# USTC3DV/D3Human-code

Measured on AMD Instinct MI355X. Metric: train iters/sec @ tet-res 128, 1024^2 render; 1/2/4/8 MI355X, higher is better.
Workload: dtype f32; 1 GPU; config3: 4-frame batch, tet-res 128 (Kuhn n=63: 262144 verts / 1500282 tets), 1024x1024, mask+normal+SSIM+sdf_reg+eikonal; frames_per_gpu=4, mesh_faces=8626, parallelism=frame-parallel dp1

## Files before the change

d3human-code_amd/csrc/raster.hip:

```cpp
#include "d3h_common.h"
#include "composite.h"

namespace {

struct TriSetup {
    float X[3], Y[3], q[3], zw[3];
    bool ok;
    bool cross;
};

__device__ __forceinline__ TriSetup load_tri(const float* __restrict__ pos, const int* __restrict__ tri, int f) {
    TriSetup t;
    int nfront = 0;
#pragma unroll
    for (int k = 0; k < 3; ++k) {
        int vi = tri[3 * (size_t)f + k];
        float4 p = *(const float4*)(pos + 4 * (size_t)vi);
        if (p.w > 1e-8f) ++nfront;
        float w = (fabsf(p.w) < 1e-8f) ? ((p.w < 0.f) ? -1e-8f : 1e-8f) : p.w;
        float q = 1.0f / w;
        t.q[k] = q;
        t.X[k] = p.x * q;
        t.Y[k] = p.y * q;
        t.zw[k] = p.z * q;
    }
    t.ok = nfront == 3;
    t.cross = nfront == 1 || nfront == 2;
    return t;
}

__device__ __forceinline__ void edge_fn(const TriSetup& t, float fx, float fy, float (&a)[3]) {
    float x0 = t.X[0] - fx, y0 = t.Y[0] - fy, x1 = t.X[1] - fx, y1 = t.Y[1] - fy, x2 = t.X[2] - fx, y2 = t.Y[2] - fy;
// ... 767 lines not shown
    if (gg.g_face && d_face) {
        float* df = d_face + (size_t)b * face_bstride + (size_t)f * fw;
        for (int c = 0; c < fw; ++c) {
            float gc = hit ? gg.g_face[i * fw + c] : 0.f;
            float s = d3h_seg_sum(gc * u, lane, sg.start) + d3h_seg_sum(gc * v, lane, sg.start) + d3h_seg_sum(gc * (1.0f - u - v), lane, sg.start);
            if (sg.tail && hit && s != 0.f) atomicAdd(df + c, s);
        }
    }
    if (d_rast && inb) *(float4*)(d_rast + 4 * i) = make_float4(gu, gv, 0.f, 0.f);
    if (RAST) {
        const bool live = hit && !(gu == 0.f && gv == 0.f);
        if (__ballot(live) == 0ull) return;
        float out[9] = {0.f, 0.f, 0.f, 0.f, 0.f, 0.f, 0.f, 0.f, 0.f};
        int vi[3];
        if (live) {
            const int rem = (int)(i % npix_per_b);
            raster_bwd_pixel(pos + (size_t)b * pos_bstride, tri, f, rem % W, rem / W, H, W, gu, gv, out, vi);
        }
#pragma unroll
        for (int k = 0; k < 3; ++k) {
            const float sx = d3h_seg_sum(out[3 * k + 0], lane, sg.start);
            const float sy = d3h_seg_sum(out[3 * k + 1], lane, sg.start);
            const float sw = d3h_seg_sum(out[3 * k + 2], lane, sg.start);
            if (sg.tail && hit && (sx != 0.f || sy != 0.f || sw != 0.f)) {
                float* dp = d_pos + (size_t)b * pos_bstride + 4 * (size_t)tri[3 * (size_t)f + k];
                atomicAdd(dp + 0, sx);
                atomicAdd(dp + 1, sy);
                atomicAdd(dp + 3, sw);
            }
        }
    }
}

__device__ __forceinline__ unsigned hash64(unsigned long long k) {
    k ^= k >> 33; k *= 0xff51afd7ed558ccdull; k ^= k >> 33; k *= 0xc4ceb9fe1a85ec53ull; k ^= k >> 33;
    return (unsigned)k;
}

__global__ void aa_hash_build_kernel(const int* __restrict__ tri, int nf, unsigned long long* __restrict__ keys, int* __restrict__ vals, unsigned mask) {
    int i = blockIdx.x * blockDim.x + threadIdx.x;
    if (i >= 3 * nf) return;
    int f = i / 3, e = i % 3;
    int va = tri[3 * (size_t)f + e], vb = tri[3 * (size_t)f + (e + 1) % 3], vo = tri[3 * (size_t)f + (e + 2) % 3];
    if (va == vb) return;
    unsigned long long key = ((unsigned long long)(unsigned)min(va, vb) << 32) | (unsigned)max(va, vb);
    unsigned slot = hash64(key) & mask;
    for (unsigned probe = 0; probe <= mask; ++probe) {
        unsigned long long prev = atomicCAS(&keys[slot], ~0ull, key);
        if (prev == ~0ull || prev == key) {
            if (atomicCAS(&vals[2 * slot], -1, vo) != -1) atomicCAS(&vals[2 * slot + 1], -1, vo);
            return;
        }
        slot = (slot + 1) & mask;
    }
}

__device__ __forceinline__ int hash_other(const unsigned long long* __restrict__ keys, const int* __restrict__ vals, unsigned mask, int va, int vb,
                                          int vo) {
    unsigned long long key = ((unsigned long long)(unsigned)min(va, vb) << 32) | (unsigned)max(va, vb);
    unsigned slot = hash64(key) & mask;
    for (unsigned probe = 0; probe <= mask; ++probe) {
        unsigned long long k = keys[slot];
        if (k == key) {
            int o0 = vals[2 * slot], o1 = vals[2 * slot + 1];
            if (o1 == -1) return -1;
            return (o0 == vo) ? o1 : o0;
// ... 700 lines not shown
                       idx, nidx, n, npb, out, out_da);
    D3H_LAUNCH_CHECK();
    return D3H_OK;
}

extern "C" int d3h_interpolate_bwd_da(const float* attr, int attr_bstride, int na, const float* rast, const int* tri, const float* db,
                                      const int* idx, int nidx, const float* g_out, const float* g_da, int nb, int H, int W, float* d_attr,
                                      float* d_rast, float* d_db, void* stream) {
    if (nb < 0 || H < 0 || W < 0 || na < 0 || nidx < 0 || (!idx && nidx != na) || (g_da && !db)) return D3H_ERR_ARG;
    size_t npb = (size_t)H * W, n = npb * nb;
    if (n == 0) return D3H_OK;
    if (!rast) return D3H_ERR_ARG;
    hipLaunchKernelGGL(interp_bwd_da_kernel, dim3(d3h_cdiv(n, 256)), dim3(256), 0, (hipStream_t)stream, attr, attr_bstride, na, rast, tri, db,
                       idx, nidx, g_out, g_da, n, npb, d_attr, d_rast, d_db);
    D3H_LAUNCH_CHECK();
    return D3H_OK;
}

extern "C" int d3h_gbuffer_fwd(const float* attr, int attr_bstride, int na, const float* face_attr, int face_bstride, int fw, const float* rast,
                               const int* tri, int nb, int H, int W, float* out0, int w0, float* out1, int w1, float* out2, int w2, float* out3,
                               int w3, float* face_out, float* mask_out, void* stream) {
    if (w0 < 0 || w1 < 0 || w2 < 0 || w3 < 0 || w0 + w1 + w2 + w3 != na || (face_out && (!face_attr || fw <= 0))) return D3H_ERR_ARG;
    size_t npb = (size_t)H * W, n = npb * nb;
    if (n == 0) return D3H_OK;
    GbufOut o{{out0, out1, out2, out3}, {w0, w1, w2, w3}, face_out, mask_out};
    const int kt_ = d3h_ktime_begin(D3H_KT_GBUFFER_FWD, (long long)n, (hipStream_t)stream);
    hipLaunchKernelGGL(gbuffer_fwd_kernel, dim3(d3h_cdiv(n, 256)), dim3(256), 0, (hipStream_t)stream, attr, attr_bstride, na, face_attr,
                       face_bstride, fw, rast, tri, n, npb, o);
    d3h_ktime_end(kt_, (hipStream_t)stream);
    D3H_LAUNCH_CHECK();
    return D3H_OK;
}

extern "C" int d3h_gbuffer_bwd(const float* attr, int attr_bstride, int na, int face_bstride, int fw, const float* rast, const int* tri, int nb,
                               int H, int W, const float* g0, int w0, const float* g1, int w1, const float* g2, int w2, const float* g3, int w3,
                               const float* g_face, float* d_attr, float* d_face, float* d_rast, void* stream) {
    if (w0 < 0 || w1 < 0 || w2 < 0 || w3 < 0 || w0 + w1 + w2 + w3 != na) return D3H_ERR_ARG;
    size_t npb = (size_t)H * W, n = npb * nb;
    if (n == 0) return D3H_OK;
    GbufGrad gg{{g0, g1, g2, g3}, {w0, w1, w2, w3}, g_face};
    const int kt = d3h_ktime_begin(D3H_KT_GBUFFER_BWD, (long long)n, (hipStream_t)stream);
    hipLaunchKernelGGL((gbuffer_bwd_kernel<false>), dim3(d3h_cdiv(n, 256)), dim3(256), 0, (hipStream_t)stream, attr, attr_bstride, na, face_bstride, fw,
                       rast, tri, n, npb, gg, d_attr, d_face, d_rast, (const float*)nullptr, 0, H, W, (float*)nullptr);
    d3h_ktime_end(kt, (hipStream_t)stream);
    D3H_LAUNCH_CHECK();
    return D3H_OK;
}

extern "C" int d3h_gbuffer_raster_bwd(const float* attr, int attr_bstride, int na, int face_bstride, int fw, const float* rast, const int* tri, int nb,
                                      int H, int W, const float* g0, int w0, const float* g1, int w1, const float* g2, int w2, const float* g3, int w3,
                                      const float* g_face, float* d_attr, float* d_face, const float* pos, int pos_bstride, float* d_pos,
                                      void* stream) {
    if (w0 < 0 || w1 < 0 || w2 < 0 || w3 < 0 || w0 + w1 + w2 + w3 != na || !pos || !d_pos) return D3H_ERR_ARG;
    size_t npb = (size_t)H * W, n = npb * nb;
    if (n == 0) return D3H_OK;
    GbufGrad gg{{g0, g1, g2, g3}, {w0, w1, w2, w3}, g_face};
    const int kt = d3h_ktime_begin(D3H_KT_GBUFFER_BWD, (long long)n, (hipStream_t)stream);
    hipLaunchKernelGGL((gbuffer_bwd_kernel<true>), dim3(d3h_cdiv(n, 256)), dim3(256), 0, (hipStream_t)stream, attr, attr_bstride, na, face_bstride, fw,
                       rast, tri, n, npb, gg, d_attr, d_face, (float*)nullptr, pos, pos_bstride, H, W, d_pos);
    d3h_ktime_end(kt, (hipStream_t)stream);
    D3H_LAUNCH_CHECK();
    return D3H_OK;
}

extern "C" int d3h_antialias_hash(const int* tri, int nf, unsigned long long* keys, int* vals, int cap, void* stream) {
    if (cap <= 0 || (cap & (cap - 1))) return D3H_ERR_ARG;
    hipStream_t s = (hipStream_t)stream;
    const int kt_ = d3h_ktime_begin(D3H_KT_AA_PREP, (long long)(nf), (hipStream_t)(stream));
    if ((const char*)vals == (const char*)keys + (size_t)cap * 8) {
        (void)hipMemsetAsync(keys, 0xFF, (size_t)cap * 16, s);
    } else {
        (void)hipMemsetAsync(keys, 0xFF, (size_t)cap * 8, s);
        (void)hipMemsetAsync(vals, 0xFF, (size_t)cap * 8, s);
    }
    if (nf > 0) hipLaunchKernelGGL(aa_hash_build_kernel, dim3(d3h_cdiv(3 * (int64_t)nf, 256)), dim3(256), 0, s, tri, nf, keys, vals, (unsigned)(cap - 1));
    d3h_ktime_end(kt_, (hipStream_t)(stream));
    D3H_LAUNCH_CHECK();
    return D3H_OK;
}

extern "C" int d3h_antialias_flags(const float* pos, int pos_bstride, const int* tri, int nf, int nb, const unsigned long long* keys,
                                   const int* vals, int cap, int H, int W, unsigned char* flags, void* stream) {
    if (cap <= 0 || (cap & (cap - 1))) return D3H_ERR_ARG;
    if (nf <= 0 || nb <= 0) return D3H_OK;
    hipLaunchKernelGGL(aa_edge_flags_kernel, dim3(d3h_cdiv((int64_t)nf * nb, 256)), dim3(256), 0, (hipStream_t)stream, pos, pos_bstride, tri, nf, nb,
                       keys, vals, (unsigned)(cap - 1), H, W, flags);
    D3H_LAUNCH_CHECK();
    return D3H_OK;
}

extern "C" int d3h_antialias_fwd(const float* color, const float* rast, const float* pos, int pos_bstride, const int* tri, int nf,
                                 const unsigned char* flags, int nb, int H, int W, int C, float* out, void* stream) {
// ... 83 lines not shown
```

d3human-code_amd/csrc/texmlp.hip:

```cpp
#include <cstdlib>
#include "d3h_common.h"
#include "d3h_h2.h"

namespace {

constexpr int NL = 5, NF = 2, ENC = NL * NF;
constexpr int HID = 32, OUTC = 6;
constexpr int W1N = HID * ENC, W2N = HID * HID, W3N = OUTC * HID;

struct GridCfg {
    float scale[NL];
    int res[NL];
    int offset[NL];
    int size[NL];
};

struct TexParams {
    float b0[3], b1[3];
    float omin[OUTC], omax[OUTC];
    float in_grad_scale;
    int merge_faces;
};

__device__ __forceinline__ void encode(const GridCfg& g, const float* __restrict__ table, const float (&xn)[3], float (&enc)[ENC]) {
#pragma unroll
    for (int l = 0; l < NL; ++l) {
        float p[3], fr[3];
        int pg[3];
#pragma unroll
        for (int d = 0; d < 3; ++d) {
            p[d] = fmaf(xn[d], g.scale[l], 0.5f);
            float fl = floorf(p[d]);
            fr[d] = p[d] - fl;
            pg[d] = (int)fl;
        }
        float f0 = 0.f, f1 = 0.f;
        const int res = g.res[l];
        const float2* tab = (const float2*)table + g.offset[l];
#pragma unroll
        for (int c = 0; c < 8; ++c) {
            float w = 1.f;
            int idx = 0, stride = 1;
#pragma unroll
            for (int d = 0; d < 3; ++d) {
                int bit = (c >> d) & 1;
                w *= bit ? fr[d] : (1.f - fr[d]);
                idx += (pg[d] + bit) * stride;
                stride *= res;
            }
            if (idx >= g.size[l]) idx -= g.size[l];
            float2 v = tab[idx];
            f0 = fmaf(w, v.x, f0);
            f1 = fmaf(w, v.y, f1);
        }
        enc[2 * l] = f0;
        enc[2 * l + 1] = f1;
    }
}

__device__ __forceinline__ bool normalise(const TexParams& tp, const float* __restrict__ x, float (&xn)[3], bool (&inside)[3]) {
#pragma unroll
    for (int d = 0; d < 3; ++d) {
        float v = (x[d] - tp.b0[d]) / (tp.b1[d] - tp.b0[d]);
        inside[d] = (v >= 0.f && v <= 1.f);
        xn[d] = fminf(fmaxf(v, 0.f), 1.f);
    }
    return true;
}

__device__ __forceinline__ void mlp_fwd(const float* sw, const float (&enc)[ENC], float (&z1)[HID], float (&z2)[HID], float (&o)[OUTC]) {
    const float* w1 = sw;
    const float* w2 = sw + W1N;
    const float* w3 = sw + W1N + W2N;
#pragma unroll
    for (int i = 0; i < HID; ++i) {
        float a = 0.f;
#pragma unroll
        for (int j = 0; j < ENC; ++j) a = fmaf(w1[i * ENC + j], enc[j], a);
        z1[i] = a;
    }
#pragma unroll
    for (int i = 0; i < HID; ++i) {
        float a = 0.f;
#pragma unroll
        for (int j = 0; j < HID; ++j) a = fmaf(w2[i * HID + j], fmaxf(z1[j], 0.f), a);
        z2[i] = a;
    }
#pragma unroll
    for (int i = 0; i < OUTC; ++i) {
// ... 512 lines not shown
        float* red = &sT[0][0][0];
#pragma unroll
        for (int r = 0; r < 16; ++r) {
            const int row = (r & 3) + 8 * (r >> 2) + 4 * (lane >> 5), col = lane & 31;
            red[(wave * 3 + 0) * 1024 + row * 32 + col] = acc1[r];
            red[(wave * 3 + 1) * 1024 + row * 32 + col] = acc2[r];
            red[(wave * 3 + 2) * 1024 + row * 32 + col] = acc3[r];
        }
        __syncthreads();
        for (int k = threadIdx.x; k < 3 * 1024; k += 256) {
            const int which = k >> 10, rc = k & 1023, row = rc >> 5, col = rc & 31;
            const float v = red[k] + red[3 * 1024 + k] + red[6 * 1024 + k] + red[9 * 1024 + k];
            if (v == 0.f) continue;
            if (which == 0) { if (col < ENC) atomicAdd(&d_w[row * ENC + col], v); }
            else if (which == 1) atomicAdd(&d_w[W1N + row * HID + col], v);
            else { if (row < OUTC) atomicAdd(&d_w[W1N + W2N + row * HID + col], v); }
        }
    }
}

constexpr int HP = 36;

__device__ __forceinline__ void tex_h2_image_put(float* T, const f32x16& v, int n, int h) {
#pragma unroll
    for (int r = 0; r < 16; ++r) T[rho(r, h) * HP + n] = v[r];
}
__device__ __forceinline__ D3hH2Frag tex_h2_image_frag(const float* T, int row, int s, int kh) {
    const float* p = T + row * HP + 16 * s + 8 * kh;
    const f32x4 a = *(const f32x4*)p, b = *(const f32x4*)(p + 4);
    const float v[8] = {a[0], a[1], a[2], a[3], b[0], b[1], b[2], b[3]};
    return d3h_h2_frag(v);
}

__global__ __launch_bounds__(512) void texmlp_bwd_mlp_h2_kernel(GridCfg g, TexParams tp, const float* __restrict__ x, const float* __restrict__ mask,
                                                                const float* __restrict__ table, const float* __restrict__ w, int64_t n,
                                                                const float* __restrict__ g_out, float* __restrict__ d_w, float* __restrict__ genc) {
    __shared__ __attribute__((aligned(16))) float smem[8 * 2 * 32 * HP];
    static_assert(4 * 3 * 1024 <= 8 * 2 * 32 * HP, "the flush buffer lives in the images");
#ifndef D3H_EMULATED
    asm volatile("v_mov_b32 v255, 0" ::: "v255");
#endif
    const int wave = threadIdx.x >> 6, lane = threadIdx.x & 63, m = lane & 31, h = lane >> 5;
    float* TA = smem + (wave * 2 + 0) * 32 * HP;
    float* TB = smem + (wave * 2 + 1) * 32 * HP;
    const float* w1 = w;
    const float* w2 = w + W1N;
    const float* w3 = w + W1N + W2N;
    __shared__ __attribute__((aligned(16))) d3h_u32x4 sA[10][2][64];
    if (wave == 0) {
        auto put = [&](int slot, const float (&v)[8]) {
            const D3hH2Frag f = d3h_h2_frag(v);
            sA[slot][0][lane] = f.h;
            sA[slot][1][lane] = f.m;
        };
        float v[8];
#pragma unroll
        for (int j = 0; j < 8; ++j) v[j] = (8 * h + j < ENC) ? w1[m * ENC + 8 * h + j] : 0.f;
        put(0, v);
#pragma unroll
        for (int j = 0; j < 8; ++j) v[j] = (8 * h + j < OUTC) ? w3[(8 * h + j) * HID + m] : 0.f;
        put(1, v);
#pragma unroll
        for (int s = 0; s < 2; ++s) {
#pragma unroll
            for (int j = 0; j < 8; ++j) v[j] = w2[m * HID + rho(8 * s + j, h)];
            put(2 + s, v);
#pragma unroll
            for (int j = 0; j < 8; ++j) v[j] = (m < OUTC) ? w3[m * HID + rho(8 * s + j, h)] : 0.f;
            put(4 + s, v);
#pragma unroll
            for (int j = 0; j < 8; ++j) v[j] = w2[rho(8 * s + j, h) * HID + m];
            put(6 + s, v);
#pragma unroll
            for (int j = 0; j < 8; ++j) v[j] = (m < ENC) ? w1[rho(8 * s + j, h) * ENC + m] : 0.f;
            put(8 + s, v);
        }
    }
    __syncthreads();
    auto Aw = [&](int slot) { D3hH2Frag f; f.h = sA[slot][0][lane]; f.m = sA[slot][1][lane]; return f; };
    f32x16 acc1, acc2, acc3;
#pragma unroll
    for (int r = 0; r < 16; ++r) { acc1[r] = 0.f; acc2[r] = 0.f; acc3[r] = 0.f; }
    const f32x16 zero16 = acc1;
    const int64_t nwt = (n + 63) / 64;
    for (int64_t wt = (int64_t)blockIdx.x * 8 + wave; wt < nwt; wt += (int64_t)gridDim.x * 8) {
        const int64_t p0 = wt * 64;
        const int64_t i = p0 + lane;
        const bool active = (i < n) && !(mask && !(mask[i] > 0.f));
        const unsigned long long am = __ballot(active);
        if (am == 0ull) continue;
        float xn[3] = {0.f, 0.f, 0.f}, enc[ENC];
        bool inside[3] = {false, false, false};
#pragma unroll
        for (int c = 0; c < ENC; ++c) enc[c] = 0.f;
        if (active) {
            normalise(tp, x + 3 * i, xn, inside);
            encode(g, table, xn, enc);
        }
        float eo[ENC];
#pragma unroll
        for (int c = 0; c < ENC; ++c) eo[c] = __shfl_xor(enc[c], 32);
#pragma unroll 1
        for (int ch = 0; ch < 2; ++ch) {
            if (((am >> (32 * ch)) & 0xffffffffull) == 0ull) continue;
            const bool own = (h == ch);
            float b8[8];
#pragma unroll
            for (int j = 0; j < 8; ++j) {
                const float e_own = (j < ENC) ? enc[j < ENC ? j : 0] : 0.f, e_oth = (j < ENC) ? eo[j < ENC ? j : 0] : 0.f;
                const float f_own = (8 + j < ENC) ? enc[8 + j < ENC ? 8 + j : 0] : 0.f, f_oth = (8 + j < ENC) ? eo[8 + j < ENC ? 8 + j : 0] : 0.f;
                b8[j] = (h == 0) ? (own ? e_own : e_oth) : (own ? f_own : f_oth);
            }
            const D3hH2Frag Benc = d3h_h2_frag(b8);
            f32x16 hi = zero16, lo = zero16;
            d3h_h2_mac32(hi, lo, Aw(0), Benc);
            const f32x16 Z1 = d3h_h2_fold(hi, lo);
            hi = zero16; lo = zero16;
#pragma unroll
            for (int s = 0; s < 2; ++s) {
#pragma unroll
                for (int j = 0; j < 8; ++j) b8[j] = fmaxf(Z1[8 * s + j], 0.f);
                d3h_h2_mac32(hi, lo, Aw(2 + s), d3h_h2_frag(b8));
            }
            const f32x16 Z2 = d3h_h2_fold(hi, lo);
            hi = zero16; lo = zero16;
#pragma unroll
            for (int s = 0; s < 2; ++s) {
#pragma unroll
                for (int j = 0; j < 8; ++j) b8[j] = fmaxf(Z2[8 * s + j], 0.f);
                d3h_h2_mac32(hi, lo, Aw(4 + s), d3h_h2_frag(b8));
            }
            const f32x16 Z3 = d3h_h2_fold(hi, lo);
            const int64_t pp = p0 + 32 * ch + m;
            const bool pact = (am >> (32 * ch + m)) & 1ull;
            float go[4] = {0.f, 0.f, 0.f, 0.f};
            float gmax = 0.f;
#pragma unroll
            for (int r = 0; r < 4; ++r) {
                const int c = r + 4 * h;
                if (c < OUTC && pact) {
                    const float sg = 1.f / (1.f + expf(-Z3[r]));
                    go[r] = g_out[pp * OUTC + c] * (tp.omax[c] - tp.omin[c]) * sg * (1.f - sg);
                    const float a = fabsf(go[r]);
                    gmax = (a < 3.0e38f) ? fmaxf(gmax, a) : gmax;
                }
            }
#pragma unroll
            for (int k = 32; k > 0; k >>= 1) gmax = fmaxf(gmax, __shfl_xor(gmax, k));
            if (!(gmax > 0.f)) {
                if (pact) {
#pragma unroll
                    for (int r = 0; r < 16; ++r) {
                        const int row = rho(r, h);
                        if (row < ENC) genc[pp * ENC + row] = 0.f;
                    }
                }
                continue;
            }
            const float S = d3h_h2_pow2_scale(gmax), Si = 1.0f / S;
#pragma unroll
            for (int r = 0; r < 4; ++r) go[r] *= S;
            const float g4 = __shfl_xor(go[0], 32), g5 = __shfl_xor(go[1], 32);
            {
                const float v[8] = {h == 0 ? go[0] : 0.f, h == 0 ? go[1] : 0.f, h == 0 ? go[2] : 0.f, h == 0 ? go[3] : 0.f, h == 0 ? g4 : 0.f, h == 0 ? g5 : 0.f, 0.f, 0.f};
                hi = zero16; lo = zero16;
                d3h_h2_mac32(hi, lo, Aw(1), d3h_h2_frag(v));
            }
            f32x16 GZ2 = d3h_h2_fold(hi, lo);
#pragma unroll
            for (int r = 0; r < 16; ++r) GZ2[r] = (Z2[r] > 0.f) ? GZ2[r] : 0.f;
            hi = zero16; lo = zero16;
#pragma unroll
            for (int s = 0; s < 2; ++s) {
#pragma unroll
                for (int j = 0; j < 8; ++j) b8[j] = GZ2[8 * s + j];
                d3h_h2_mac32(hi, lo, Aw(6 + s), d3h_h2_frag(b8));
            }
            f32x16 GZ1 = d3h_h2_fold(hi, lo);
#pragma unroll
            for (int r = 0; r < 16; ++r) GZ1[r] = (Z1[r] > 0.f) ? GZ1[r] : 0.f;
            hi = zero16; lo = zero16;
#pragma unroll
            for (int s = 0; s < 2; ++s) {
#pragma unroll
                for (int j = 0; j < 8; ++j) b8[j] = GZ1[8 * s + j];
                d3h_h2_mac32(hi, lo, Aw(8 + s), d3h_h2_frag(b8));
            }
            const f32x16 GE = d3h_h2_fold(hi, lo);
            if (pact) {
                const float sc = tp.in_grad_scale * Si;
#pragma unroll
                for (int r = 0; r < 16; ++r) {
                    const int row = rho(r, h);
                    if (row < ENC) genc[pp * ENC + row] = GE[r] * sc;
                }
            }
            if (d_w) {
                auto outer = [&](f32x16& acc) {
                    f32x16 th = zero16, tl = zero16;
#pragma unroll
                    for (int s = 0; s < 2; ++s) d3h_h2_mac32(th, tl, tex_h2_image_frag(TA, m, s, h), tex_h2_image_frag(TB, m, s, h));
#pragma unroll
                    for (int r = 0; r < 16; ++r) acc[r] = fmaf(fmaf(tl[r], D3H_H2_INV_SCALE, th[r]), Si, acc[r]);
                };
                f32x16 gov = zero16, t16;
#pragma unroll
                for (int r = 0; r < 4; ++r) gov[r] = (r + 4 * h < OUTC) ? go[r] : 0.f;
                tex_h2_image_put(TA, gov, m, h);
#pragma unroll
                for (int r = 0; r < 16; ++r) t16[r] = pact ? fmaxf(Z2[r], 0.f) : 0.f;
                tex_h2_image_put(TB, t16, m, h);
                D3H_WAVE_SYNC();
                outer(acc3);
                D3H_WAVE_SYNC();
                tex_h2_image_put(TA, GZ2, m, h);
#pragma unroll
                for (int r = 0; r < 16; ++r) t16[r] = pact ? fmaxf(Z1[r], 0.f) : 0.f;
                tex_h2_image_put(TB, t16, m, h);
                D3H_WAVE_SYNC();
                outer(acc2);
                D3H_WAVE_SYNC();
                tex_h2_image_put(TA, GZ1, m, h);
#pragma unroll
                for (int r = 0; r < 16; ++r) {
                    const int row = rho(r, h);
                    float e = 0.f;
#pragma unroll
// ... 79 lines not shown
    return tp;
}

}

extern "C" int64_t d3h_hashgrid_param_floats(double per_level_scale, int base_res) {
    GridCfg g = make_cfg(per_level_scale, base_res);
    long long last = (long long)g.res[NL - 1] * g.res[NL - 1] * g.res[NL - 1];
    last = (last + 7) / 8 * 8;
    return ((int64_t)g.offset[NL - 1] + last) * NF;
}

extern "C" int d3h_texmlp_fwd(const float* x, const float* mask, const float* table, const float* w, int64_t n, double per_level_scale,
                              int base_res, const float* bbox, const float* omin, const float* omax, float* out, float* enc_out, void* stream) {
    if (n < 0 || !bbox) return D3H_ERR_ARG;
    if (n == 0) return D3H_OK;
    GridCfg g = make_cfg(per_level_scale, base_res);
    TexParams tp = make_tp(bbox, omin, omax, 1.f);
    const int kt = d3h_ktime_begin(D3H_KT_TEX_FWD, n, (hipStream_t)stream);
    const int64_t ntile = (n + 255) / 256;
    const unsigned grid = (unsigned)(ntile < (1 << 20) ? ntile : (1 << 20));
    if (out && w && !enc_out)
        hipLaunchKernelGGL(texmlp_fwd_mfma_kernel, dim3(grid < 2039u ? grid : 2039u), dim3(256), 0, (hipStream_t)stream, g, tp, x, mask, table, w, n, out);
    else
        hipLaunchKernelGGL(texmlp_fwd_kernel, dim3(grid), dim3(256), 0, (hipStream_t)stream, g, tp, x, mask, table, w, n, out, enc_out);
    d3h_ktime_end(kt, (hipStream_t)stream);
    D3H_LAUNCH_CHECK();
    return D3H_OK;
}

extern "C" int d3h_texmlp_bwd(const float* x, const float* mask, const float* table, const float* w, int64_t n, double per_level_scale,
                              int base_res, const float* bbox, const float* omin, const float* omax, float in_grad_scale, int enc_only,
                              const float* g_out, float* d_table, float* d_w, float* d_x, float* genc_scratch, void* stream) {
    if (n < 0 || !bbox) return D3H_ERR_ARG;
    if (n == 0) return D3H_OK;
    GridCfg g = make_cfg(per_level_scale, base_res);
    TexParams tp = make_tp(bbox, omin, omax, in_grad_scale);
    int64_t ntile = (n + 255) / 256;
    int grid = (int)(ntile < 1021 ? ntile : 1021);
    hipStream_t s = (hipStream_t)stream;
    float* nof = nullptr;
    if (enc_only) {
        const int kt = d3h_ktime_begin(D3H_KT_TEX_BWD_ENC, n, s);
        hipLaunchKernelGGL((texmlp_bwd_kernel<1>), dim3(grid), dim3(256), 0, s, g, tp, x, mask, table, w, n, g_out, d_table, d_w, d_x, nof);
        d3h_ktime_end(kt, s);
    } else if (genc_scratch) {
        int grid2 = (int)(ntile < 4093 ? ntile : 4093);
        int gridm = (int)(ntile < 509 ? ntile : 509);
        const int ktm = d3h_ktime_begin(D3H_KT_TEX_BWD_MLP, n, s);
        static int tex_h2 = -1;
        if (tex_h2 < 0) { const char* e = getenv("D3H_TEX_H2"); tex_h2 = (e && e[0] == '0') ? 0 : 1; }
        const int64_t nwt8 = (n + 511) / 512;
        if (tex_h2) hipLaunchKernelGGL(texmlp_bwd_mlp_h2_kernel, dim3((unsigned)(nwt8 < 251 ? nwt8 : 251)), dim3(512), 0, s, g, tp, x, mask, table, w, n, g_out, d_w, genc_scratch);
        else hipLaunchKernelGGL(texmlp_bwd_mlp_kernel, dim3(gridm), dim3(256), 0, s, g, tp, x, mask, table, w, n, g_out, d_w, genc_scratch);
        d3h_ktime_end(ktm, s);
        if (d_table || d_x) {
            const int kte = d3h_ktime_begin(D3H_KT_TEX_BWD_ENC, n, s);
            hipLaunchKernelGGL((texmlp_bwd_kernel<1>), dim3(grid2), dim3(256), 0, s, g, tp, x, mask, table, w, n, (const float*)genc_scratch, d_table, nof, d_x,
                               nof);
            d3h_ktime_end(kte, s);
        }
    } else {
        hipLaunchKernelGGL((texmlp_bwd_kernel<0>), dim3(grid), dim3(256), 0, s, g, tp, x, mask, table, w, n, g_out, d_table, d_w, d_x, nof);
    }
    D3H_LAUNCH_CHECK();
    return D3H_OK;
}
```

d3human-code_amd/d3h/texmlp.py:

```python
import ctypes
import os
import math
import weakref

import torch
from d3h._lib import cur_stream as _cur_stream

from . import _lib as L
from . import gradarena as _GA

PER_LEVEL_SCALE = math.exp(math.log(4096 / 16) / (16 - 1))
BASE_RES = 16
N_LEVELS, N_FEATURES = 5, 2
ENC_DIMS = N_LEVELS * N_FEATURES


def grid_param_count(per_level_scale=PER_LEVEL_SCALE, base_res=BASE_RES):
    return int(L.lib().d3h_hashgrid_param_floats(ctypes.c_double(per_level_scale), L.i32(base_res)))


def _f6(v):
    return (ctypes.c_float * 6)(*[float(x) for x in v])


ASYNC_TABLE_GRAD = os.environ.get('D3H_ASYNC_TABLE_GRAD', '1') != '0'
_SIDE = {}
_PENDING = []
_PASS = {'table_grad_returned': False, 'callback': False}


def _scatter_stream(t):
    if not t.is_cuda or L.emulated():
        return None
    s = _SIDE.get(t.device)
    if s is None:
        s = _SIDE[t.device] = torch.cuda.Stream(device=t.device)
    return s


def _join_scatter():
    while _PENDING:
        _cur_stream().wait_stream(_PENDING.pop())


def _end_of_pass():
    _join_scatter()
    _PASS['table_grad_returned'] = False
    _PASS['callback'] = False


def _mark_table_grad_returned():
    _PASS['table_grad_returned'] = True
    if not _PASS['callback']:
        _PASS['callback'] = True
        torch.autograd.Variable._execution_engine.queue_callback(_end_of_pass)


class _TexMLPFn(torch.autograd.Function):
# ... 23 lines not shown
        need_tab, need_w, need_x = ctx.needs_input_grad[2], any(ctx.needs_input_grad[3:6]), ctx.needs_input_grad[0]
        leaf = ctx.table_leaf() if ctx.table_leaf is not None else None
        wl, ctx.w_leaves = ctx.w_leaves, None
        d_tab = d_tab_ret = d_w = None
        w_ret = True
        first_contribution = not _PASS['table_grad_returned'] and leaf is not None and leaf.grad is None
        if need_tab:
            d_tab = d_tab_ret = _GA.slot_for(leaf) if tab.data_ptr() == (leaf.data_ptr() if leaf is not None else 0) else None
            if d_tab is None:
                d_tab = _GA.accum_for(leaf)
                if d_tab is None:
                    d_tab = d_tab_ret = L.zeros_like(tab)
        if need_w:
            if wl is not None and all(ctx.needs_input_grad[3:6]):
                d_w = _GA.block_for(wl)
                if d_w is None:
                    d_w = _GA.accum_block_for(wl)
                    w_ret = d_w is None
            if d_w is None:
                d_w = L.zeros_like(wcat)
        d_x = torch.empty_like(xs) if need_x else None
        genc = torch.empty(n, 10, dtype=torch.float32, device=xs.device)
        gc = g.reshape(-1, 6).contiguous().float()
        mp = m if has_mask else None
        args = lambda: (L.ptr(xs), L.ptr(mp), L.ptr(tab), L.ptr(wcat), L.i64(n), ctypes.c_double(PER_LEVEL_SCALE), L.i32(BASE_RES), _f6(bbox),
                        _f6(omin), _f6(omax), L.f32(gs))
        side = _scatter_stream(xs) if (ASYNC_TABLE_GRAD and need_tab and need_x and first_contribution) else None
        if side is None:
            _join_scatter()
            L.check(lib.d3h_texmlp_bwd(*args(), L.i32(0), L.ptr(gc), L.ptr(d_tab), L.ptr(d_w), L.ptr(d_x), L.ptr(genc), L.stream()), 'texmlp_bwd')
        else:
            main = _cur_stream()
            _join_scatter()
            L.check(lib.d3h_texmlp_bwd(*args(), L.i32(0), L.ptr(gc), None, L.ptr(d_w), None, L.ptr(genc), L.stream()), 'texmlp_bwd_mlp')
            L.check(lib.d3h_texmlp_bwd(*args(), L.i32(1), L.ptr(genc), None, None, L.ptr(d_x), None, L.stream()), 'texmlp_bwd_dx')
            side.wait_stream(main)
            with L.use_stream(side):
                L.check(lib.d3h_texmlp_bwd(*args(), L.i32(1), L.ptr(genc), L.ptr(d_tab), None, None, None, L.stream()), 'texmlp_bwd_table')
            for t in (xs, tab, genc, d_tab) + ((mp,) if mp is not None else ()):
                t.record_stream(side)
            _PENDING.append(side)
        if need_tab:
            _mark_table_grad_returned()
        if d_w is not None and w_ret:
            n1, n2 = s1.numel(), s2.numel()
            dw1, dw2, dw3 = d_w[:n1].reshape(s1), d_w[n1:n1 + n2].reshape(s2), d_w[n1 + n2:].reshape(s3)
        else:
            dw1 = dw2 = dw3 = None
        return (d_x.reshape(xshape) if d_x is not None else None, None, d_tab_ret, dw1, dw2, dw3, None, None, None, None)


def texture_mlp(x, table, w1, w2, w3, bbox, omin, omax, mask=None, in_grad_scale=128.0):
    return _TexMLPFn.apply(x, mask, table, w1, w2, w3, tuple(float(v) for v in bbox), tuple(float(v) for v in omin),
                           tuple(float(v) for v in omax), in_grad_scale)


class _GridEncodeFn(torch.autograd.Function):
    @staticmethod
    def forward(ctx, x, table):
        xs = x.reshape(-1, 3).contiguous().float()
        n = xs.shape[0]
        tab = table.contiguous().float()
        enc = torch.empty(n, ENC_DIMS, dtype=torch.float32, device=x.device)
        unit = (0.0, 0.0, 0.0, 1.0, 1.0, 1.0)
        L.check(L.lib().d3h_texmlp_fwd(L.ptr(xs), None, L.ptr(tab), None, L.i64(n), ctypes.c_double(PER_LEVEL_SCALE), L.i32(BASE_RES), _f6(unit),
                                       None, None, None, L.ptr(enc), L.stream()), 'hashgrid_fwd')
        ctx.save_for_backward(xs, tab)
        ctx.xshape = x.shape
# ... 20 lines not shown
```

Before: 238.2 iters/s.

## Add tiled LDS-aggregated gbuffer backward and fuse texture dx into MLP backward

Replaces the flat per-pixel gbuffer backward with a 2D-tiled kernel. It skips empty tiles and accumulates per-vertex and per-face gradients in a small shared-memory hash before flushing to global atomics, which cuts global atomic contention. Separately, the texture MLP backward kernel now computes the hash-grid spatial derivative inline and writes d_x directly, removing a second encode pass and kernel launch. The costs are more LDS use per block, which can lower occupancy, and extra code paths behind environment switches.

Measured after the change: 252.3 iters/s (median of 6 runs). 1.06x the previous value.

```diff
diff --git a/d3human-code_amd/csrc/raster.hip b/d3human-code_amd/csrc/raster.hip
--- a/d3human-code_amd/csrc/raster.hip
+++ b/d3human-code_amd/csrc/raster.hip
@@ -1,3 +1,6 @@
+#include <algorithm>
+#include <cstdlib>
+#include <cstring>
 #include "d3h_common.h"
 #include "composite.h"
 
@@ -831,6 +834,184 @@
     }
 }
 
+constexpr int GBL_VCAP = 256, GBL_VPOOL = 4096;
+constexpr int GBL_FCAP = 256, GBL_FPOOL = 1024;
+constexpr int GBL_PROBES = 8;
+constexpr int GBL_SLOTS = 64;
+
+__device__ __forceinline__ int gbl_claim(int* keys, int cap, int key) {
+    if (cap == 0) return -1;
+    int s = (int)(((unsigned)key * 0x9E3779B1u) >> 16) & (cap - 1);
+    for (int p = 0; p < GBL_PROBES && p < cap; ++p) {
+        const int old = atomicCAS(&keys[s], -1, key);
+        if (old == -1 || old == key) return s;
+        s = (s + 1) & (cap - 1);
+    }
+    return -1;
+}
+
+template <bool RAST, int TW, int TH>
+__global__ __launch_bounds__(256) void gbuffer_bwd_tile_kernel(const float* __restrict__ attr, int attr_bstride, int na, int face_bstride, int fw,
+                                                               const float* __restrict__ rast, const int* __restrict__ tri, GbufGrad gg,
+                                                               float* __restrict__ d_attr, float* __restrict__ d_face, float* __restrict__ d_rast,
+                                                               const float* __restrict__ pos, int pos_bstride, int H, int W,
+                                                               float* __restrict__ d_pos, int vcap, int fcap) {
+    static_assert((TW * TH) % 256 == 0 && TW <= 256 && 256 % TW == 0, "a pass of the workgroup covers whole tile rows");
+    __shared__ __attribute__((aligned(16))) float vval[GBL_VPOOL];
+    __shared__ __attribute__((aligned(16))) float fval[GBL_FPOOL];
+    __shared__ int vkey[GBL_VCAP];
+    __shared__ int fkey[GBL_FCAP];
+    const int tid = threadIdx.x, lane = tid & 63;
+    const int b = blockIdx.z;
+    const int na_v = d_attr ? na : 0;
+    const int vstride = na_v + (RAST ? 3 : 0);
+    const bool want_face = gg.g_face && d_face;
+    __shared__ int s_any;
+    if (tid == 0) s_any = 0;
+    __syncthreads();
+    {
+        bool any = false;
+        for (int pass = 0; pass < TW * TH / 256; ++pass) {
+            const int lp = pass * 256 + tid;
+            const int px = blockIdx.x * TW + lp % TW, py = blockIdx.y * TH + lp / TW;
+            if (px < W && py < H) any = any || rast[4 * (((size_t)b * H + py) * W + px) + 3] > 0.f;
+        }
+        if (any) s_any = 1;
+    }
+    __syncthreads();
+    if (!s_any) {
+        if (d_rast) {
+            for (int pass = 0; pass < TW * TH / 256; ++pass) {
+                const int lp = pass * 256 + tid;
+                const int px = blockIdx.x * TW + lp % TW, py = blockIdx.y * TH + lp / TW;
+                if (px < W && py < H) *(float4*)(d_rast + 4 * (((size_t)b * H + py) * W + px)) = make_float4(0.f, 0.f, 0.f, 0.f);
+            }
+        }
+        return;
+    }
+    for (int k = tid; k < vcap; k += 256) vkey[k] = -1;
+    for (int k = 4 * tid; k < vcap * vstride; k += 1024) *(float4*)&vval[k] = make_float4(0.f, 0.f, 0.f, 0.f);
+    if (want_face) {
+        for (int k = tid; k < fcap; k += 256) fkey[k] = -1;
+        for (int k = 4 * tid; k < fcap * fw; k += 1024) *(float4*)&fval[k] = make_float4(0.f, 0.f, 0.f, 0.f);
+    }
+    __syncthreads();
+    const float* ab = attr + (size_t)b * attr_bstride;
+    float* db_ = d_attr ? d_attr + (size_t)b * attr_bstride : nullptr;
+    float* dfb = want_face ? d_face + (size_t)b * face_bstride : nullptr;
+    float* dpb = RAST ? d_pos + (size_t)b * pos_bstride : nullptr;
+#pragma unroll 1
+    for (int pass = 0; pass < TW * TH / 256; ++pass) {
+        const int lp = pass * 256 + tid;
+        const int px = blockIdx.x * TW + lp % TW, py = blockIdx.y * TH + lp / TW;
+        const bool inb = px < W && py < H;
+        const size_t i = ((size_t)b * H + (inb ? py : 0)) * W + (inb ? px : 0);
+        float4 r = inb ? *(const float4*)(rast + 4 * i) : make_float4(0.f, 0.f, 0.f, 0.f);
+        const int id = (int)r.w;
+        const bool hit = id > 0;
+        if (__ballot(hit) == 0ull) {
+            if (d_rast && inb) *(float4*)(d_rast + 4 * i) = make_float4(0.f, 0.f, 0.f, 0.f);
+            continue;
+        }
+        const D3hSeg sg = d3h_seg_runs(hit ? id : -1, lane);
+        const bool tail = sg.tail && hit;
+        float gu = 0.f, gv = 0.f;
+        const int f = hit ? id - 1 : 0;
+        int vi[3] = {0, 0, 0};
+        if (hit) { vi[0] = tri[3 * (size_t)f]; vi[1] = tri[3 * (size_t)f + 1]; vi[2] = tri[3 * (size_t)f + 2]; }
+        const size_t i0 = (size_t)vi[0] * na, i1 = (size_t)vi[1] * na, i2 = (size_t)vi[2] * na;
+        int sl[3] = {-1, -1, -1};
+        if (tail && vstride > 0) {
+#pragma unroll
+            for (int k = 0; k < 3; ++k) sl[k] = gbl_claim(vkey, vcap, vi[k]);
+        }
+        const float u = r.x, v = r.y;
+        int c0 = 0;
+#pragma unroll
+        for (int g = 0; g < GBUF_GROUPS; ++g) {
+            const int wd = gg.width[g];
+            if (gg.g[g]) {
+                for (int c = 0; c < wd; ++c) {
+                    float gc = hit ? gg.g[g][i * wd + c] : 0.f;
+                    const int ch = c0 + c;
+                    if (db_) {
+                        float s0 = d3h_seg_sum(gc * u, lane, sg.start);
+                        float s1 = d3h_seg_sum(gc * v, lane, sg.start);
+                        float s2 = d3h_seg_sum(gc * (1.0f - u - v), lane, sg.start);
+                        if (tail) {
+                            if (s0 != 0.f) { if (sl[0] >= 0) atomicAdd(&vval[sl[0] * vstride + ch], s0); else atomicAdd(db_ + i0 + ch, s0); }
+                            if (s1 != 0.f) { if (sl[1] >= 0) atomicAdd(&vval[sl[1] * vstride + ch], s1); else atomicAdd(db_ + i1 + ch, s1); }
+                            if (s2 != 0.f) { if (sl[2] >= 0) atomicAdd(&vval[sl[2] * vstride + ch], s2); else atomicAdd(db_ + i2 + ch, s2); }
+                        }
+                    }
+                    if (hit && gc != 0.f) {
+                        float x2 = ab[i2 + ch];
+                        gu = fmaf(gc, ab[i0 + ch] - x2, gu);
+                        gv = fmaf(gc, ab[i1 + ch] - x2, gv);
+                    }
+                }
+            }
+            c0 += wd;
+        }
+        if (want_face) {
+            const int sf = tail ? gbl_claim(fkey, fcap, f) : -1;
+            for (int c = 0; c < fw; ++c) {
+                float gc = hit ? gg.g_face[i * fw + c] : 0.f;
+                float s = d3h_seg_sum(gc * u, lane, sg.start) + d3h_seg_sum(gc * v, lane, sg.start) + d3h_seg_sum(gc * (1.0f - u - v), lane, sg.start);
+                if (tail && s != 0.f) { if (sf >= 0) atomicAdd(&fval[sf * fw + c], s); else atomicAdd(dfb + (size_t)f * fw + c, s); }
+            }
+        }
+        if (d_rast && inb) *(float4*)(d_rast + 4 * i) = make_float4(gu, gv, 0.f, 0.f);
+        if (RAST) {
+            const bool live = hit && !(gu == 0.f && gv == 0.f);
+            if (__ballot(live) == 0ull) continue;
+            float out[9] = {0.f, 0.f, 0.f, 0.f, 0.f, 0.f, 0.f, 0.f, 0.f};
+            int vj[3];
+            if (live) raster_bwd_pixel(pos + (size_t)b * pos_bstride, tri, f, px, py, H, W, gu, gv, out, vj);
+#pragma unroll
+            for (int k = 0; k < 3; ++k) {
+                const float sx = d3h_seg_sum(out[3 * k + 0], lane, sg.start);
+                const float sy = d3h_seg_sum(out[3 * k + 1], lane, sg.start);
+                const float sw = d3h_seg_sum(out[3 * k + 2], lane, sg.start);
+                if (tail && (sx != 0.f || sy != 0.f || sw != 0.f)) {
+                    if (sl[k] >= 0) {
+                        float* dv = &vval[sl[k] * vstride + na_v];
+                        atomicAdd(dv + 0, sx);
+                        atomicAdd(dv + 1, sy);
+                        atomicAdd(dv + 2, sw);
+                    } else {
+                        float* dp = dpb + 4 * (size_t)vi[k];
+                        atomicAdd(dp + 0, sx);
+                        atomicAdd(dp + 1, sy);
+                        atomicAdd(dp + 3, sw);
+                    }
+                }
+            }
+        }
+    }
+    __syncthreads();
+    for (int k = tid; k < vcap * 16; k += 256) {
+        const int slot = k >> 4, key = vkey[slot];
+        if (key < 0) continue;
+        for (int c = k & 15; c < vstride; c += 16) {
+            const float s = vval[slot * vstride + c];
+            if (s == 0.f) continue;
+            if (c < na_v) atomicAdd(db_ + (size_t)key * na + c, s);
+            else if (RAST) atomicAdd(dpb + 4 * (size_t)key + (c - na_v == 2 ? 3 : c - na_v), s);
+        }
+    }
+    if (want_face) {
+        for (int k = tid; k < fcap * 4; k += 256) {
+            const int slot = k >> 2, key = fkey[slot];
+            if (key < 0) continue;
+            for (int c = k & 3; c < fw; c += 4) {
+                const float s = fval[slot * fw + c];
+                if (s != 0.f) atomicAdd(dfb + (size_t)key * fw + c, s);
+            }
+        }
+    }
+}
+
 __device__ __forceinline__ unsigned hash64(unsigned long long k) {
     k ^= k >> 33; k *= 0xff51afd7ed558ccdull; k ^= k >> 33; k *= 0xc4ceb9fe1a85ec53ull; k ^= k >> 33;
     return (unsigned)k;
@@ -1597,6 +1778,32 @@
     return D3H_OK;
 }
 
+static inline int gbl_pow2_floor(int v) { int p = 0; for (int q = 1; q > 0 && q <= v; q <<= 1) p = q; return p; }
+template <bool RAST>
+static bool gbuffer_bwd_tile_launch(const float* attr, int attr_bstride, int na, int face_bstride, int fw, const float* rast, const int* tri, int nb,
+                                    int H, int W, const GbufGrad& gg, float* d_attr, float* d_face, float* d_rast, const float* pos, int pos_bstride,
+                                    float* d_pos, hipStream_t s) {
+    const char* e = getenv("D3H_GBUF_LDS");
+    if ((e && e[0] == '0') || nb > 65535) return false;
+    e = getenv("D3H_GBUF_LDS_SLOTS");
+    const int limit = e ? atoi(e) : GBL_SLOTS;
+    const int vstride = (d_attr ? na : 0) + (RAST ? 3 : 0);
+    const int vcap = (vstride > 0 && limit > 0) ? gbl_pow2_floor(std::min(std::min(limit, GBL_VCAP), GBL_VPOOL / vstride)) : 0;
+    const int fcap = (fw > 0 && limit > 0) ? gbl_pow2_floor(std::min(std::min(limit, GBL_FCAP), GBL_FPOOL / fw)) : 0;
+    e = getenv("D3H_GBUF_TILE");
+    const int tw = e ? atoi(e) : 16, th = (e && strchr(e, 'x')) ? atoi(strchr(e, 'x') + 1) : 16;
+#define GBL_LAUNCH(TW, TH)                                                                                                                         \
+    hipLaunchKernelGGL((gbuffer_bwd_tile_kernel<RAST, TW, TH>), dim3(d3h_cdiv(W, TW), d3h_cdiv(H, TH), nb), dim3(256), 0, s, attr, attr_bstride, na, \
+                       face_bstride, fw, rast, tri, gg, d_attr, d_face, d_rast, pos, pos_bstride, H, W, d_pos, vcap, fcap)
+    if (tw == 64 && th == 4) GBL_LAUNCH(64, 4);
+    else if (tw == 8 && th == 32) GBL_LAUNCH(8, 32);
+    else if (tw == 32 && th == 32) GBL_LAUNCH(32, 32);
+    else if (tw == 32 && th == 8) GBL_LAUNCH(32, 8);
+    else GBL_LAUNCH(16, 16);
+#undef GBL_LAUNCH
+    return true;
+}
+
 extern "C" int d3h_gbuffer_bwd(const float* attr, int attr_bstride, int na, int face_bstride, int fw, const float* rast, const int* tri, int nb,
                                int H, int W, const float* g0, int w0, const float* g1, int w1, const float* g2, int w2, const float* g3, int w3,
                                const float* g_face, float* d_attr, float* d_face, float* d_rast, void* stream) {
@@ -1605,8 +1812,10 @@
     if (n == 0) return D3H_OK;
     GbufGrad gg{{g0, g1, g2, g3}, {w0, w1, w2, w3}, g_face};
     const int kt = d3h_ktime_begin(D3H_KT_GBUFFER_BWD, (long long)n, (hipStream_t)stream);
-    hipLaunchKernelGGL((gbuffer_bwd_kernel<false>), dim3(d3h_cdiv(n, 256)), dim3(256), 0, (hipStream_t)stream, attr, attr_bstride, na, face_bstride, fw,
-                       rast, tri, n, npb, gg, d_attr, d_face, d_rast, (const float*)nullptr, 0, H, W, (float*)nullptr);
+    if (!gbuffer_bwd_tile_launch<false>(attr, attr_bstride, na, face_bstride, fw, rast, tri, nb, H, W, gg, d_attr, d_face, d_rast, nullptr, 0, nullptr,
+                                        (hipStream_t)stream))
+        hipLaunchKernelGGL((gbuffer_bwd_kernel<false>), dim3(d3h_cdiv(n, 256)), dim3(256), 0, (hipStream_t)stream, attr, attr_bstride, na, face_bstride,
+                           fw, rast, tri, n, npb, gg, d_attr, d_face, d_rast, (const float*)nullptr, 0, H, W, (float*)nullptr);
     d3h_ktime_end(kt, (hipStream_t)stream);
     D3H_LAUNCH_CHECK();
     return D3H_OK;
@@ -1621,8 +1830,10 @@
     if (n == 0) return D3H_OK;
     GbufGrad gg{{g0, g1, g2, g3}, {w0, w1, w2, w3}, g_face};
     const int kt = d3h_ktime_begin(D3H_KT_GBUFFER_BWD, (long long)n, (hipStream_t)stream);
-    hipLaunchKernelGGL((gbuffer_bwd_kernel<true>), dim3(d3h_cdiv(n, 256)), dim3(256), 0, (hipStream_t)stream, attr, attr_bstride, na, face_bstride, fw,
-                       rast, tri, n, npb, gg, d_attr, d_face, (float*)nullptr, pos, pos_bstride, H, W, d_pos);
+    if (!gbuffer_bwd_tile_launch<true>(attr, attr_bstride, na, face_bstride, fw, rast, tri, nb, H, W, gg, d_attr, d_face, nullptr, pos, pos_bstride, d_pos,
+                                       (hipStream_t)stream))
+        hipLaunchKernelGGL((gbuffer_bwd_kernel<true>), dim3(d3h_cdiv(n, 256)), dim3(256), 0, (hipStream_t)stream, attr, attr_bstride, na, face_bstride,
+                           fw, rast, tri, n, npb, gg, d_attr, d_face, (float*)nullptr, pos, pos_bstride, H, W, d_pos);
     d3h_ktime_end(kt, (hipStream_t)stream);
     D3H_LAUNCH_CHECK();
     return D3H_OK;
diff --git a/d3human-code_amd/csrc/texmlp.hip b/d3human-code_amd/csrc/texmlp.hip
--- a/d3human-code_amd/csrc/texmlp.hip
+++ b/d3human-code_amd/csrc/texmlp.hip
@@ -55,6 +55,54 @@
         }
         enc[2 * l] = f0;
         enc[2 * l + 1] = f1;
+    }
+}
+
+__device__ __forceinline__ void encode_dx(const GridCfg& g, const float* __restrict__ table, const float (&xn)[3], const float (&ins)[3],
+                                          float (&enc)[ENC], float* dE) {
+#pragma unroll
+    for (int l = 0; l < NL; ++l) {
+        float p[3], fr[3];
+        int pg[3];
+#pragma unroll
+        for (int d = 0; d < 3; ++d) {
+            p[d] = fmaf(xn[d], g.scale[l], 0.5f);
+            float fl = floorf(p[d]);
+            fr[d] = p[d] - fl;
+            pg[d] = (int)fl;
+        }
+        float f0 = 0.f, f1 = 0.f, d0[3] = {0.f, 0.f, 0.f}, d1[3] = {0.f, 0.f, 0.f};
+        const int res = g.res[l];
+        const float2* tab = (const float2*)table;
+#pragma unroll
+        for (int c = 0; c < 8; ++c) {
+            float w = 1.f, wd[3];
+            int idx = 0, stride = 1;
+#pragma unroll
+            for (int d = 0; d < 3; ++d) {
+                int bit = (c >> d) & 1;
+                wd[d] = bit ? fr[d] : (1.f - fr[d]);
+                w *= wd[d];
+                idx += (pg[d] + bit) * stride;
+                stride *= res;
+            }
+            if (idx >= g.size[l]) idx -= g.size[l];
+            float2 v = tab[g.offset[l] + idx];
+            f0 = fmaf(w, v.x, f0);
+            f1 = fmaf(w, v.y, f1);
+            const float dw[3] = {(c & 1) ? wd[1] * wd[2] : -(wd[1] * wd[2]), (c & 2) ? wd[0] * wd[2] : -(wd[0] * wd[2]),
+                                 (c & 4) ? wd[0] * wd[1] : -(wd[0] * wd[1])};
+#pragma unroll
+            for (int d = 0; d < 3; ++d) { d0[d] = fmaf(dw[d], v.x, d0[d]); d1[d] = fmaf(dw[d], v.y, d1[d]); }
+        }
+        enc[2 * l] = f0;
+        enc[2 * l + 1] = f1;
+#pragma unroll
+        for (int d = 0; d < 3; ++d) {
+            const float s = g.scale[l] * ins[d];
+            dE[(3 * (2 * l) + d) * 64] = d0[d] * s;
+            dE[(3 * (2 * l + 1) + d) * 64] = d1[d] * s;
+        }
     }
 }
 
@@ -633,15 +681,18 @@
     return d3h_h2_frag(v);
 }
 
+template <bool DX>
 __global__ __launch_bounds__(512) void texmlp_bwd_mlp_h2_kernel(GridCfg g, TexParams tp, const float* __restrict__ x, const float* __restrict__ mask,
                                                                 const float* __restrict__ table, const float* __restrict__ w, int64_t n,
-                                                                const float* __restrict__ g_out, float* __restrict__ d_w, float* __restrict__ genc) {
+                                                                const float* __restrict__ g_out, float* __restrict__ d_w, float* __restrict__ genc,
+                                                                float* __restrict__ d_x) {
     __shared__ __attribute__((aligned(16))) float smem[8 * 2 * 32 * HP];
     static_assert(4 * 3 * 1024 <= 8 * 2 * 32 * HP, "the flush buffer lives in the images");
+    __shared__ float sDE[DX ? 8 : 1][DX ? 3 * ENC * 64 : 1];
 #ifndef D3H_EMULATED
     asm volatile("v_mov_b32 v255, 0" ::: "v255");
 #endif
-    const int wave = threadIdx.x >> 6, lane = threadIdx.x & 63, m = lane & 31, h = lane >> 5;
+    const int wave = __builtin_amdgcn_readfirstlane((int)(threadIdx.x >> 6)), lane = threadIdx.x & 63, m = lane & 31, h = lane >> 5;
     float* TA = smem + (wave * 2 + 0) * 32 * HP;
     float* TB = smem + (wave * 2 + 1) * 32 * HP;
     const float* w1 = w;
@@ -683,12 +734,20 @@
 #pragma unroll
     for (int r = 0; r < 16; ++r) { acc1[r] = 0.f; acc2[r] = 0.f; acc3[r] = 0.f; }
     const f32x16 zero16 = acc1;
-    const int64_t nwt = (n + 63) / 64;
-    for (int64_t wt = (int64_t)blockIdx.x * 8 + wave; wt < nwt; wt += (int64_t)gridDim.x * 8) {
-        const int64_t p0 = wt * 64;
+    float rng[4];
+#pragma unroll
+    for (int r = 0; r < 4; ++r) {
+        const int c1 = r + 4 < OUTC ? r + 4 : 0;
+        const float lo_half = tp.omax[r] - tp.omin[r], hi_half = r + 4 < OUTC ? tp.omax[c1] - tp.omin[c1] : 0.f;
+        rng[r] = h == 0 ? lo_half : hi_half;
+    }
+    const int nwt = (int)((n + 63) / 64);
+    for (int wt = (int)blockIdx.x * 8 + wave; wt < nwt; wt += (int)gridDim.x * 8) {
+        const int64_t p0 = (int64_t)wt * 64;
         const int64_t i = p0 + lane;
         const bool active = (i < n) && !(mask && !(mask[i] > 0.f));
         const unsigned long long am = __ballot(active);
+        if (DX && !active && i < n) { d_x[3 * i] = 0.f; d_x[3 * i + 1] = 0.f; d_x[3 * i + 2] = 0.f; }
         if (am == 0ull) continue;
         float xn[3] = {0.f, 0.f, 0.f}, enc[ENC];
         bool inside[3] = {false, false, false};
@@ -696,8 +755,14 @@
         for (int c = 0; c < ENC; ++c) enc[c] = 0.f;
         if (active) {
             normalise(tp, x + 3 * i, xn, inside);
-            encode(g, table, xn, enc);
-        }
+            if (DX) {
+                const float ins[3] = {inside[0] ? 1.f : 0.f, inside[1] ? 1.f : 0.f, inside[2] ? 1.f : 0.f};
+                encode_dx(g, table, xn, ins, enc, sDE[wave] + lane);
+            } else {
+                encode(g, table, xn, enc);
+            }
+        }
+        if (DX) D3H_WAVE_SYNC();
         float eo[ENC];
 #pragma unroll
         for (int c = 0; c < ENC; ++c) eo[c] = __shfl_xor(enc[c], 32);
@@ -741,7 +806,7 @@
                 const int c = r + 4 * h;
                 if (c < OUTC && pact) {
                     const float sg = 1.f / (1.f + expf(-Z3[r]));
-                    go[r] = g_out[pp * OUTC + c] * (tp.omax[c] - tp.omin[c]) * sg * (1.f - sg);
+                    go[r] = g_out[pp * OUTC + c] * rng[r] * sg * (1.f - sg);
                     const float a = fabsf(go[r]);
                     gmax = (a < 3.0e38f) ? fmaxf(gmax, a) : gmax;
                 }
@@ -755,6 +820,7 @@
                         const int row = rho(r, h);
                         if (row < ENC) genc[pp * ENC + row] = 0.f;
                     }
+                    if (DX && h == 0) { d_x[3 * pp] = 0.f; d_x[3 * pp + 1] = 0.f; d_x[3 * pp + 2] = 0.f; }
                 }
                 continue;
             }
@@ -794,6 +860,25 @@
                 for (int r = 0; r < 16; ++r) {
                     const int row = rho(r, h);
                     if (row < ENC) genc[pp * ENC + row] = GE[r] * sc;
+                }
+            }
+            if (DX) {
+                const float* dE = sDE[wave] + 32 * ch + m;
+                const float sc = tp.in_grad_scale * Si;
+                float gx[3] = {0.f, 0.f, 0.f};
+                static_assert(ENC == 10, "the row split below");
+#pragma unroll
+                for (int r = 0; r < 6; ++r) {
+                    const int row = r < 4 ? r + 4 * h : 4 + r;
+                    const float ge = (pact && (r < 4 || h == 0)) ? GE[r] * sc : 0.f;
+#pragma unroll
+                    for (int d = 0; d < 3; ++d) gx[d] = fmaf(dE[(3 * row + d) * 64], ge, gx[d]);
+                }
+#pragma unroll
+                for (int d = 0; d < 3; ++d) gx[d] += __shfl_xor(gx[d], 32);
+                if (pact && h == 0) {
+#pragma unroll
+                    for (int d = 0; d < 3; ++d) d_x[3 * pp + d] = gx[d] / (tp.b1[d] - tp.b0[d]);
                 }
             }
             if (d_w) {
@@ -939,7 +1024,7 @@
 extern "C" int d3h_texmlp_bwd(const float* x, const float* mask, const float* table, const float* w, int64_t n, double per_level_scale,
                               int base_res, const float* bbox, const float* omin, const float* omax, float in_grad_scale, int enc_only,
                               const float* g_out, float* d_table, float* d_w, float* d_x, float* genc_scratch, void* stream) {
-    if (n < 0 || !bbox) return D3H_ERR_ARG;
+    if (n < 0 || n >= ((int64_t)1 << 36) || !bbox) return D3H_ERR_ARG;
     if (n == 0) return D3H_OK;
     GridCfg g = make_cfg(per_level_scale, base_res);
     TexParams tp = make_tp(bbox, omin, omax, in_grad_scale);
@@ -958,9 +1043,13 @@
         static int tex_h2 = -1;
         if (tex_h2 < 0) { const char* e = getenv("D3H_TEX_H2"); tex_h2 = (e && e[0] == '0') ? 0 : 1; }
         const int64_t nwt8 = (n + 511) / 512;
-        if (tex_h2) hipLaunchKernelGGL(texmlp_bwd_mlp_h2_kernel, dim3((unsigned)(nwt8 < 251 ? nwt8 : 251)), dim3(512), 0, s, g, tp, x, mask, table, w, n, g_out, d_w, genc_scratch);
+        const char* ef = getenv("D3H_TEX_DX_FUSED");
+        float* d_x_mlp = (tex_h2 && !(ef && ef[0] == '0')) ? d_x : nullptr;
+        if (tex_h2 && d_x_mlp) hipLaunchKernelGGL((texmlp_bwd_mlp_h2_kernel<true>), dim3((unsigned)(nwt8 < 251 ? nwt8 : 251)), dim3(512), 0, s, g, tp, x, mask, table, w, n, g_out, d_w, genc_scratch, d_x_mlp);
+        else if (tex_h2) hipLaunchKernelGGL((texmlp_bwd_mlp_h2_kernel<false>), dim3((unsigned)(nwt8 < 251 ? nwt8 : 251)), dim3(512), 0, s, g, tp, x, mask, table, w, n, g_out, d_w, genc_scratch, nof);
         else hipLaunchKernelGGL(texmlp_bwd_mlp_kernel, dim3(gridm), dim3(256), 0, s, g, tp, x, mask, table, w, n, g_out, d_w, genc_scratch);
         d3h_ktime_end(ktm, s);
+        if (d_x_mlp) d_x = nullptr;
         if (d_table || d_x) {
             const int kte = d3h_ktime_begin(D3H_KT_TEX_BWD_ENC, n, s);
             hipLaunchKernelGGL((texmlp_bwd_kernel<1>), dim3(grid2), dim3(256), 0, s, g, tp, x, mask, table, w, n, (const float*)genc_scratch, d_table, nof, d_x,
diff --git a/d3human-code_amd/d3h/texmlp.py b/d3human-code_amd/d3h/texmlp.py
--- a/d3human-code_amd/d3h/texmlp.py
+++ b/d3human-code_amd/d3h/texmlp.py
@@ -24,6 +24,7 @@
 
 
 ASYNC_TABLE_GRAD = os.environ.get('D3H_ASYNC_TABLE_GRAD', '1') != '0'
+DX_FUSED = os.environ.get('D3H_TEX_DX_FUSED', '1') != '0'
 _SIDE = {}
 _PENDING = []
 _PASS = {'table_grad_returned': False, 'callback': False}
@@ -113,8 +114,11 @@
         else:
             main = _cur_stream()
             _join_scatter()
-            L.check(lib.d3h_texmlp_bwd(*args(), L.i32(0), L.ptr(gc), None, L.ptr(d_w), None, L.ptr(genc), L.stream()), 'texmlp_bwd_mlp')
-            L.check(lib.d3h_texmlp_bwd(*args(), L.i32(1), L.ptr(genc), None, None, L.ptr(d_x), None, L.stream()), 'texmlp_bwd_dx')
+            if DX_FUSED:
+                L.check(lib.d3h_texmlp_bwd(*args(), L.i32(0), L.ptr(gc), None, L.ptr(d_w), L.ptr(d_x), L.ptr(genc), L.stream()), 'texmlp_bwd_mlp_dx')
+            else:
+                L.check(lib.d3h_texmlp_bwd(*args(), L.i32(0), L.ptr(gc), None, L.ptr(d_w), None, L.ptr(genc), L.stream()), 'texmlp_bwd_mlp')
+                L.check(lib.d3h_texmlp_bwd(*args(), L.i32(1), L.ptr(genc), None, None, L.ptr(d_x), None, L.stream()), 'texmlp_bwd_dx')
             side.wait_stream(main)
             with L.use_stream(side):
                 L.check(lib.d3h_texmlp_bwd(*args(), L.i32(1), L.ptr(genc), L.ptr(d_tab), None, None, None, L.stream()), 'texmlp_bwd_table')
```
